# cwchenwang/outdoor-nerf-depth

Hardware: AMD Instinct MI355X
Metric: train rays/sec, KITTI 375x1242, 64+128 samples/ray (higher is better)
Workload: dtype bf16 MFMA operands, f32 accumulate / f32 master weights

## Files before the change

outdoor_nerf_depth_amd/csrc/nerfpp_common.h:

```cpp
#pragma once
#include <stdint.h>
#ifdef NERFPP_PROBES
#include <stdlib.h>
#endif

namespace nerfpp {

constexpr int WIDTH = 256;
constexpr int FRAG_BYTES = 1024;
constexpr int BLK_FRAGS = 16;
constexpr int DIR_REF = 27;
constexpr int DIRW = 32;
constexpr int N_NET = 2;

__host__ __device__ constexpr int pe_dim(int net) { return net == 0 ? 3 : 4; }
__host__ __device__ constexpr int pe_ref_ch(int net) { return net == 0 ? 63 : 84; }
__host__ __device__ constexpr int kpe(int net) { return net == 0 ? 4 : 6; }
__host__ __device__ constexpr int kpew(int net) { return kpe(net) * 16; }

enum RefTensor { RT_L0 = 0, RT_SIGMA = 8, RT_REMAP = 9, RT_RGB0 = 10, RT_RGB1 = 11, RT_COUNT = 12 };
__host__ __device__ constexpr int ref_out(int t) {
  return t < 8 ? 256 : t == RT_SIGMA ? 1 : t == RT_REMAP ? 256 : t == RT_RGB0 ? 128 : 3;
}
__host__ __device__ constexpr int ref_in(int net, int t) {
// ... 19 lines not shown
__host__ __device__ constexpr int fs_nkc(int net, int s) {
  return s == FS_L0 ? kpe(net) : s == FS_L5 ? kpe(net) + 16 : s == FS_REMAP ? 0 : s < FS_REMAP ? 16
       : s == FS_SIG ? 16 : s == FS_RGB0 ? 20 : 16;
}
constexpr int DERIVED_WC = 128 * 256;
constexpr int DERIVED_FLOATS = DERIVED_WC + 128;
__host__ __device__ constexpr int fs_frags(int net, int s) { return fs_nob(s) * fs_nkc(net, s); }
__host__ __device__ constexpr int fs_frag_off(int net, int s) {
  int off = 0;
  for (int i = 0; i < s; ++i) off += fs_frags(net, i);
  return off;
}
__host__ __device__ constexpr int fs_bias_off(int s) {
  int off = 0;
  for (int i = 0; i < s; ++i) off += fs_nob(i) * 32;
  return off;
}
__host__ __device__ constexpr int fwd_frags(int net) { return fs_frag_off(net, FS_COUNT); }
constexpr int FWD_BIAS_FLOATS = fs_bias_off(FS_COUNT);
static_assert(fwd_frags(0) % BLK_FRAGS == 0 && fwd_frags(1) % BLK_FRAGS == 0, "block aligned");

enum BwdStage { BS_DG = 0, BS_DR = 1, BS_DH7 = 2, BS_COUNT = 10 };
__host__ __device__ constexpr int bs_nob(int s) { return s == BS_DG ? 4 : 8; }
__host__ __device__ constexpr int bs_nkc(int s) { return s == BS_DG ? 4 : s == BS_DR ? 0 : s == BS_DH7 ? 10 : 16; }
__host__ __device__ constexpr int bs_frags(int s) { return bs_nob(s) * bs_nkc(s); }
__host__ __device__ constexpr int bs_frag_off(int s) {
  int off = 0;
  for (int i = 0; i < s; ++i) off += bs_frags(i);
  return off;
}
constexpr int BWD_FRAGS = bs_frag_off(BS_COUNT);
static_assert(BWD_FRAGS % BLK_FRAGS == 0, "block aligned");
__host__ __device__ constexpr int bs_layer(int s) { return 10 - s; }

__host__ __device__ constexpr int w_planes(int P) { return P == 1 ? 1 : 2; }
__host__ __device__ constexpr int a_planes(int P) { return P == 2 ? 2 : 1; }
__host__ __device__ constexpr size_t fwd_stream_bytes(int net, int P) { return (size_t)fwd_frags(net) * FRAG_BYTES * w_planes(P); }
__host__ __device__ constexpr size_t bwd_stream_bytes(int P) { return (size_t)BWD_FRAGS * FRAG_BYTES * w_planes(P); }

__host__ __device__ constexpr int kslot(int c, int hi, int t) { return 16 * c + 8 * (t >> 2) + 4 * hi + (t & 3); }
__host__ __device__ constexpr int dfeat(int ob, int hi, int r) { return ob * 32 + (r & 3) + 8 * (r >> 2) + 4 * hi; }

__host__ __device__ constexpr int pe_ref_of_lane_slot(int D, int hi, int m) {
  const int nf = 10 * D;
  if (m < nf) {
    const int k = 5 * hi + m / (2 * D), d = (m % (2 * D)) / 2, s = m & 1;
    return D + k * 2 * D + s * D + d;
  }
  const int id = 2 * hi + (m - nf);
  return (m - nf) < 2 && id < D ? id : -1;
}
__host__ __device__ constexpr int dir_ref_of_lane_slot(int hi, int m) {
  if (m < 12) {
    const int k = 2 * hi + m / 6, d = (m % 6) / 2, s = m & 1;
    return 3 + k * 6 + s * 3 + d;
  }
  const int id = 2 * hi + (m - 12);
  return (m - 12) < 2 && id < 3 ? id : -1;
}
__host__ __device__ constexpr int feat_hi(int f) { return ((f % 16) / 4) % 2; }
__host__ __device__ constexpr int feat_m(int f) { return 8 * (f / 16) + 4 * ((f % 16) / 8) + (f % 4); }
__host__ __device__ constexpr int pe_ref_of_feat(int net, int f) { return pe_ref_of_lane_slot(pe_dim(net), feat_hi(f), feat_m(f)); }
__host__ __device__ constexpr int dir_ref_of_feat(int f) { return dir_ref_of_lane_slot(feat_hi(f), feat_m(f)); }

enum Tensor {
  T_X = 0, T_H0 = 1,  T_R = 9, T_G = 10, T_DIRX = 11,
// ... 211 lines not shown
```

outdoor_nerf_depth_amd/csrc/nerfpp_mlp.hip:

```cpp
#include <hip/hip_runtime.h>
#include <math.h>
#include <stdint.h>
#include <type_traits>
#include <utility>
#include "hip_device.h"
#include "nerfpp_common.h"
#include "nerfpp_kernels.h"

#ifdef NERFPP_PROBES
#include "nerfpp_mlp_probes.h"
#else
namespace nerfpp { namespace probe {
constexpr int STAMP_BYTES = 0;
__device__ __forceinline__ void stamp(int, int, int, int, uint32_t) {}
__device__ __forceinline__ void dump_stamps(uint32_t, int, int) {}
}}
#endif

namespace nerfpp {

using hipdev::bf16x8, hipdev::bf16x2, hipdev::f16x8, hipdev::f16x2, hipdev::f32x2, hipdev::f32x4, hipdev::f32x8, hipdev::f32x16;
using hipdev::u32x4, hipdev::s16x2, hipdev::s16x8, hipdev::glds16xN_saddr;
#define LDS_AS __attribute__((address_space(3)))

template <int P> struct Frag { bf16x8 v[a_planes(P)]; };

extern __shared__ __attribute__((aligned(16))) char smem[];

enum { PIPE_RING = 1, PIPE_ROLES = 2 };

__device__ __forceinline__ uint32_t lds_base_addr() { return (uint32_t)(uintptr_t)(LDS_AS char*)smem; }

template <int P, int NW, int MODE, int NBUF, int BF = BLK_FRAGS>
struct WeightPipe {
  static constexpr int BLKF = BF;
  static constexpr int BLK_BYTES = BF * P * FRAG_BYTES;
  static constexpr int SHARE = MODE == PIPE_ROLES ? BF * P : BF * P / NW;
  static constexpr int AHEAD = NBUF - 1;
  static_assert(AHEAD >= 1 && AHEAD <= 3 && (AHEAD - 1) * SHARE < 63, "ring depth");
  const char* g;
  uint32_t stamp_off = 0;
  int nblk, cur, step, wave, lane;
  int slot_cur, slot_issue, next_issue;
  uint32_t lds_base;
  __device__ __forceinline__ void init(const void* stream, int nblk_, int wave_, int lane_) {
    g = (const char*)stream; nblk = nblk_; cur = 0; step = 0; wave = wave_; lane = lane_;
    slot_cur = 0; slot_issue = 0; next_issue = 0;
    lds_base = lds_base_addr();
#pragma unroll
    for (int b = 0; b < AHEAD; ++b) issue();
  }
  static constexpr bool TRICKLE = MODE == PIPE_RING && AHEAD >= 2;
  int pend_blk = -1, pend_slot = 0;
  __device__ __forceinline__ void issue_frags(int blk, int slot, int f0, int f1) {
    if (MODE == PIPE_ROLES && wave != 0) return;
    const int w0 = MODE == PIPE_ROLES ? 0 : wave * SHARE;
    const char* sb = g + (size_t)blk * BLK_BYTES + (size_t)w0 * FRAG_BYTES;
    const uint32_t dst = lds_base + slot * BLK_BYTES + w0 * FRAG_BYTES;
#pragma unroll
    for (int f = f0; f < f1; f += 4) {
      const int n = f1 - f < 4 ? f1 - f : 4;
      const char* a = sb + f * FRAG_BYTES;
      const uint32_t d = dst + f * FRAG_BYTES;
      if (n == 4) glds16xN_saddr<4>(a, (uint32_t)lane * 16u, d);
      else if (n == 3) glds16xN_saddr<3>(a, (uint32_t)lane * 16u, d);
      else if (n == 2) glds16xN_saddr<2>(a, (uint32_t)lane * 16u, d);
      else glds16xN_saddr<1>(a, (uint32_t)lane * 16u, d);
    }
  }
  __device__ __forceinline__ bool claim(int& blk, int& slot) {
    blk = next_issue; slot = slot_issue;
    ++next_issue;
    slot_issue = slot_issue + 1 == NBUF ? 0 : slot_issue + 1;
    return blk < nblk;
  }
  __device__ __forceinline__ void issue() {
    int blk, slot;
    if (!claim(blk, slot)) return;
    static_assert(SHARE == 2 || SHARE % 4 == 0, "per-wave fragment count");
    issue_frags(blk, slot, 0, SHARE);
  }
  __device__ __forceinline__ void trickle(int i, int n) {
    if constexpr (TRICKLE) {
      if (pend_blk < 0) return;
      issue_frags(pend_blk, pend_slot, SHARE * i / n, SHARE * (i + 1) / n);
    }
  }
  __device__ __forceinline__ void wait_counted() {
    const int younger = nblk - 1 - step < AHEAD - 1 ? nblk - 1 - step : AHEAD - 1;
    if (AHEAD >= 3 && younger >= 2) asm volatile("s_waitcnt vmcnt(%0)" ::"n"(2 * SHARE) : "memory");
    else if (AHEAD >= 2 && younger == 1) asm volatile("s_waitcnt vmcnt(%0)" ::"n"(SHARE) : "memory");
// ... 73 lines not shown
          const f16x8 bf = __builtin_bit_cast(f16x8, b[blk * KPB + kl].v[0]);
#pragma unroll
          for (int g = 0; g < G; ++g) acc[ob + g] = __builtin_amdgcn_mfma_f32_32x32x16_f16(__builtin_bit_cast(f16x8, wh[g]), bf, acc[ob + g], 0, 0, 0);
#pragma unroll
          for (int g = 0; g < G; ++g) acc[ob + g] = __builtin_amdgcn_mfma_f32_32x32x16_f16(__builtin_bit_cast(f16x8, wl[g]), bf, acc[ob + g], 0, 0, 0);
          pipe.trickle(kl * UPB + ob / G, KPB * UPB);
        }
      } else {
#pragma unroll
        for (int ob = 0; ob < NOB; ++ob) {
          mfma_p<P>(acc[ob], l + (kl * NOB + ob) * w_planes(P) * FRAG_BYTES, b[blk * KPB + kl]);
          if (UPB == 2 && (ob & 3) == 3) pipe.trickle(kl * 2 + (ob >> 2), KPB * 2);
        }
        if (UPB == 1) pipe.trickle(kl, KPB);
      }
    }
    hook(blk);
    const int live_kl = LIVE - blk * KPB < KPB ? (LIVE - blk * KPB < 0 ? 0 : LIVE - blk * KPB) : KPB;
    constexpr int W = w_planes(P), D = P == 1 ? LDS_PREFETCH : LDS_PREFETCH_SPLIT;
    const int N = NOB * live_kl;
    if (N < D) continue;
#pragma unroll
    for (int i = 0; i < D; ++i) __builtin_amdgcn_sched_group_barrier(0x100, W, 0);
#pragma unroll
    for (int i = 0; i < N - D; ++i) {
      __builtin_amdgcn_sched_group_barrier(0x008, W, 0);
      __builtin_amdgcn_sched_group_barrier(0x100, W, 0);
    }
#pragma unroll
    for (int i = 0; i < D; ++i) __builtin_amdgcn_sched_group_barrier(0x008, W, 0);
  }
}

template <int P>
__device__ __forceinline__ void set_slot(Frag<P>& f, int t, float v) {
  if constexpr (P == 3) {
    f16x8 q = __builtin_bit_cast(f16x8, f.v[0]);
    q[t] = (_Float16)v;
    f.v[0] = __builtin_bit_cast(bf16x8, q);
    return;
  }
  const __bf16 h = (__bf16)v;
  f.v[0][t] = h;
  if constexpr (P == 2) f.v[1][t] = (__bf16)(v - (float)h);
}
template <int P>
__device__ __forceinline__ uint4 saved_image(const uint4 regs) {
  if constexpr (P == 3) {
    const f32x8 f = __builtin_convertvector(__builtin_bit_cast(f16x8, regs), f32x8);
    return __builtin_bit_cast(uint4, __builtin_convertvector(f, bf16x8));
  } else return regs;
}
template <int P>
__device__ __forceinline__ Frag<P> zero_frag() {
  Frag<P> f;
#pragma unroll
  for (int p = 0; p < a_planes(P); ++p)
#pragma unroll
    for (int t = 0; t < 8; ++t) f.v[p][t] = (__bf16)0.f;
  return f;
}

template <int N, int P>
__device__ __forceinline__ void stash_frags(char* base, int lane, const Frag<P> (&f)[N]) {
#pragma unroll
  for (int c = 0; c < N; ++c)
#pragma unroll
    for (int p = 0; p < a_planes(P); ++p) *(uint4*)(base + ((c * a_planes(P) + p) * 64 + lane) * 16) = *(const uint4*)&f[c].v[p];
}
template <int N, int P>
__device__ __forceinline__ void unstash_frags(const char* base, int lane, Frag<P> (&f)[N]) {
#pragma unroll
  for (int c = 0; c < N; ++c)
#pragma unroll
    for (int p = 0; p < a_planes(P); ++p) *(uint4*)&f[c].v[p] = *(const uint4*)(base + ((c * a_planes(P) + p) * 64 + lane) * 16);
}

template <int P>
__device__ __forceinline__ uint32_t pack2(float a, float b) {
  const f32x2 v = {a, b};
  if constexpr (P == 3) return __builtin_bit_cast(uint32_t, __builtin_convertvector(v, f16x2));
  else return __builtin_bit_cast(uint32_t, __builtin_convertvector(v, bf16x2));
}

template <int NOB, int P>
__device__ __forceinline__ uint4 acc_to_frags_relu_bits(const f32x16 (&acc)[NOB], Frag<P> (&h)[2 * NOB]) {
  static_assert(P == 1 || P == 3, "one operand plane");
  uint32_t m[4] = {0, 0, 0, 0};
#pragma unroll
  for (int ob = 0; ob < NOB; ++ob)
#pragma unroll
    for (int hh = 0; hh < 2; ++hh) {
      u32x4 d;
#pragma unroll
      for (int w = 0; w < 4; ++w) d[w] = pack2<P>(acc[ob][8 * hh + 2 * w], acc[ob][8 * hh + 2 * w + 1]);
#pragma unroll
      for (int w = 0; w < 4; ++w) {
        const int j = (ob & 1) * 8 + hh * 4 + w;
        asm("v_and_or_b32 %0, %1, %2, %0" : "+v"(m[ob >> 1]) : "v"(d[w] >> j), "s"(0x80008000u >> j));
      }
      const s16x8 zero = {0, 0, 0, 0, 0, 0, 0, 0};
      h[2 * ob + hh].v[0] = __builtin_bit_cast(bf16x8, __builtin_elementwise_max(__builtin_bit_cast(s16x8, d), zero));
    }
  return make_uint4(m[0], m[1], m[2], m[3]);
}

template <int N, int P>
__device__ __forceinline__ void zero_invalid(Frag<P> (&f)[N], bool valid) {
#pragma unroll
  for (int c = 0; c < N; ++c)
#pragma unroll
    for (int p = 0; p < a_planes(P); ++p) {
      u32x4 d = __builtin_bit_cast(u32x4, f[c].v[p]);
#pragma unroll
      for (int w = 0; w < 4; ++w) d[w] = valid ? d[w] : 0u;
      f[c].v[p] = __builtin_bit_cast(bf16x8, d);
    }
}

template <int NOB>
__device__ __forceinline__ void init_bias_lds(f32x16 (&acc)[NOB], uint32_t lds_off_bytes, int hi) {
  LDS_AS char* base = (LDS_AS char*)smem;
#pragma unroll
  for (int ob = 0; ob < NOB; ++ob) {
#pragma unroll
    for (int q = 0; q < 4; ++q) {
      const f32x4 v = *(LDS_AS f32x4*)(base + lds_off_bytes + (ob * 32 + hi * 16 + 4 * q) * 4);
      acc[ob][4 * q] = v[0]; acc[ob][4 * q + 1] = v[1]; acc[ob][4 * q + 2] = v[2]; acc[ob][4 * q + 3] = v[3];
    }
  }
}
template <int NOB>
__device__ __forceinline__ void init_zero(f32x16 (&acc)[NOB]) {
#pragma unroll
  for (int ob = 0; ob < NOB; ++ob)
#pragma unroll
    for (int r = 0; r < 16; ++r) acc[ob][r] = 0.f;
}

__device__ __forceinline__ void store_nt16(char* gptr, const uint4 v) {
  const u32x4 vv = {v.x, v.y, v.z, v.w};
  __builtin_nontemporal_store(vv, (u32x4*)gptr);
}

constexpr int REGION_MASK = 16 * FRAG_BYTES;
constexpr int REGION_BYTES = REGION_MASK + 1024;

__device__ __forceinline__ char* frag_addr(__bf16* base, int ld, size_t wave_row0, int c, int lane) {
  const size_t blk = (wave_row0 >> 5) * (size_t)(ld >> 4) + (size_t)c;
  return (char*)base + blk * FRAG_BYTES + ((((lane & 31) << 1) | (lane >> 5)) << 4);
}
template <int P>
__device__ __forceinline__ void store_chunk(__bf16* base, size_t plane, int ld, size_t wave_row0, int lane, int c, const Frag<P>& f, int np = a_planes(P)) {
#pragma unroll
  for (int p = 0; p < a_planes(P); ++p)
    if (p < np) store_nt16(frag_addr(base + p * plane, ld, wave_row0, c, lane), saved_image<P>(*(const uint4*)&f.v[p]));
}
template <int NCH, int P>
__device__ __forceinline__ void save_frags(__bf16* base, size_t plane, int ld, size_t wave_row0, int lane, const Frag<P> (&h)[NCH], int np = a_planes(P)) {
  __builtin_amdgcn_sched_barrier(0);
#pragma unroll
  for (int c = 0; c < NCH; ++c) store_chunk<P>(base, plane, ld, wave_row0, lane, c, h[c], np);
  __builtin_amdgcn_sched_barrier(0);
}

template <int NCH, int P>
__device__ __forceinline__ void handoff_write(char* region, int lane, const Frag<P> (&h)[NCH]) {
  static_assert(a_planes(P) == 1, "one plane");
#pragma unroll
  for (int c = 0; c < NCH; ++c) *(uint4*)(region + (c * 64 + lane) * 16) = *(const uint4*)&h[c].v[0];
}
template <int P>
__device__ __forceinline__ void handoff_flush_one(const char* region, int lane, __bf16* base, int ld, size_t row0, int cr, int ct) {
  static_assert(a_planes(P) == 1, "one plane");
  store_nt16(frag_addr(base, ld, row0, ct, lane), saved_image<P>(*(const uint4*)(region + (cr * 64 + lane) * 16)));
}
template <int P>
__device__ __forceinline__ void handoff_flush_chunks(const char* region, int lane, __bf16* base, int ld, size_t row0, int c0, int n) {
#pragma unroll 4
  for (int c = c0; c < c0 + n; ++c) handoff_flush_one<P>(region, lane, base, ld, row0, c, c);
}

template <int NOB>
__device__ __forceinline__ void mask_to_frags(const f32x16 (&acc)[NOB], const uint4 bits, Frag<1> (&dz)[2 * NOB]) {
  const uint32_t act[4] = {~bits.x, ~bits.y, ~bits.z, ~bits.w};
#pragma unroll
  for (int ob = 0; ob < NOB; ++ob)
#pragma unroll
    for (int hh = 0; hh < 2; ++hh) {
      u32x4 d;
#pragma unroll
      for (int w = 0; w < 4; ++w) d[w] = pack2<1>(acc[ob][8 * hh + 2 * w], acc[ob][8 * hh + 2 * w + 1]);
#pragma unroll
      for (int w = 0; w < 4; ++w) {
        const int j = (ob & 1) * 8 + hh * 4 + w;
        const s16x2 keep = __builtin_bit_cast(s16x2, act[ob >> 1] << j) >> (s16x2){15, 15};
        d[w] &= __builtin_bit_cast(uint32_t, keep);
      }
      dz[2 * ob + hh].v[0] = __builtin_bit_cast(bf16x8, d);
    }
}

template <int NET>
__device__ __forceinline__ void sample_point(const MlpGeom& gm, size_t row, int S, float (&x)[4], float (&vd)[3],
                                             float* depth_real) {
#pragma clang fp contract(off)
  const int ray = (int)(row / S);
  const float ox = gm.ray_o[ray * 3], oy = gm.ray_o[ray * 3 + 1], oz = gm.ray_o[ray * 3 + 2];
  const float dx = gm.ray_d[ray * 3], dy = gm.ray_d[ray * 3 + 1], dz = gm.ray_d[ray * 3 + 2];
  const float z = gm.z[row];
  const float dd = dx * dx + dy * dy + dz * dz;
  const float inv_n = 1.f / sqrtf(dd);
  vd[0] = dx * inv_n; vd[1] = dy * inv_n; vd[2] = dz * inv_n;
  if (NET == 0) {
    x[0] = ox + z * dx; x[1] = oy + z * dy; x[2] = oz + z * dz; x[3] = 0.f;
    *depth_real = 0.f;
  } else {
    const float d1 = -(dx * ox + dy * oy + dz * oz) / dd;
    const float mx = ox + d1 * dx, my = oy + d1 * dy, mz = oz + d1 * dz;
    const float pmn = sqrtf(mx * mx + my * my + mz * mz);
    const float d2 = sqrtf(1.f - pmn * pmn) * inv_n;
    const float sx = ox + (d1 + d2) * dx, sy = oy + (d1 + d2) * dy, sz = oz + (d1 + d2) * dz;
    float ax = oy * sz - oz * sy, ay = oz * sx - ox * sz, az = ox * sy - oy * sx;
    const float an = 1.f / sqrtf(ax * ax + ay * ay + az * az);
    ax *= an; ay *= an; az *= an;
    const float phi = asinf(pmn), theta = asinf(pmn * z);
    float sn, cs;
    sincosf(phi - theta, &sn, &cs);
    const float cx = ay * sz - az * sy, cy = az * sx - ax * sz, cz = ax * sy - ay * sx;
    const float dt = (ax * sx + ay * sy + az * sz) * (1.f - cs);
    float nx = sx * cs + cx * sn + ax * dt, ny = sy * cs + cy * sn + ay * dt, nz = sz * cs + cz * sn + az * dt;
    const float nn = 1.f / sqrtf(nx * nx + ny * ny + nz * nz);
    x[0] = nx * nn; x[1] = ny * nn; x[2] = nz * nn; x[3] = z;
// ... 91 lines not shown
  static constexpr int REGION = W;
  static constexpr int STASH = REGION + (ROLES ? REGION_BYTES : 0);
  static constexpr int BIAS = STASH + NW * kpe(NET) * a_planes(P) * 1024;
  static constexpr int TOTAL = BIAS + FWD_BIAS_FLOATS * 4;
};
template <int NW>
struct BwdLds {
  static constexpr int BF = BLK_FRAGS, NBUF = 4;
  static constexpr int W = NBUF * BF * FRAG_BYTES;
  static constexpr int REGION = W;
  static constexpr int MASKS = REGION + REGION_BYTES;
  static constexpr int TOTAL = MASKS + 2 * NW * 1024;
};

template <int NET, int P, int NW, bool TRAIN>
__device__ __forceinline__ void mlp_fwd_body(const MlpFwdArgs& a, const int bid) {
  using LD = FwdLds<NET, P, NW, TRAIN>;
  static_assert((P == 1 || P == 3) && LD::ROLES == TRAIN, "split-bf16 runs mlp_fwd_body_split");
  constexpr int KPE = kpe(NET);
  const int lane = threadIdx.x & 63, wave = __builtin_amdgcn_readfirstlane(threadIdx.x >> 6);
  const int hi = lane >> 5;
  const size_t row_raw = (size_t)bid * (NW * 32) + wave * 32 + (lane & 31);
  const bool valid = row_raw < (size_t)a.rows;
  const size_t row = valid ? row_raw : (size_t)a.rows - 1;
  const size_t plane_rows = a.rows_padded;
  const size_t wrow0 = (size_t)bid * (NW * 32) + wave * 32;
  const bool loader = TRAIN && wave == 0, partner = TRAIN && wave == 1;
  const bool tail = wrow0 + 32 > (size_t)a.rows;
  char* region = smem + LD::REGION;
  char* pe_stash = smem + LD::STASH + wave * (KPE * 1024);
  const size_t nblk32 = a.rows_padded / 32;
  uint4* mask_out = a.masks + (wrow0 / 32) * 64 + lane;

  WeightPipe<w_planes(P), NW, LD::MODE, LD::NBUF, LD::BF> pipe;
  pipe.stamp_off = LD::TOTAL;
  pipe.init(a.w_stream, fwd_frags(NET) / LD::BF, wave, lane);
  constexpr int H = NW >= 5 ? 4 : NW - 1, Q = (16 + H - 1) / H, CPB = LD::BF / 8;
  constexpr int RMASK = REGION_MASK;
  for (int i = threadIdx.x; i < FWD_BIAS_FLOATS / 4; i += NW * 64)
    *(float4*)(smem + LD::BIAS + i * 16) = ((const float4*)a.bias)[i];
  asm volatile("s_waitcnt vmcnt(0) lgkmcnt(0)" ::: "memory");
  __builtin_amdgcn_s_barrier();
  auto bias_init8 = [&](f32x16 (&acc_)[8], int off) { init_bias_lds<8>(acc_, LD::BIAS + off * 4, hi); };
  auto bias_init4 = [&](f32x16 (&acc_)[4], int off) { init_bias_lds<4>(acc_, LD::BIAS + off * 4, hi); };
  auto bias_init1 = [&](f32x16 (&acc_)[1], int off) { init_bias_lds<1>(acc_, LD::BIAS + off * 4, hi); };
  const size_t tile_row0 = wrow0 - (size_t)wave * 32;
  auto flush = [&](int blk, auto nch_c, __bf16* base, int ld, int mask_stage) __attribute__((always_inline)) {
    if constexpr (TRAIN) {
      constexpr int NCH = decltype(nch_c)::value;
      if (blk == 0 && wave >= 1 && wave <= H) {
#pragma unroll
        for (int c = 0; c < NCH; ++c)
          if ((c % H) == wave - 1) handoff_flush_chunks<P>(region, lane, base, ld, tile_row0, c, 1);
        if (partner && mask_stage >= 0)
          mask_out[(size_t)mask_stage * nblk32 * 64 - 64] = *(const uint4*)(region + RMASK + lane * 16);
      }
    }
  };
  auto finish_h = [&](Frag<P> (&frags)[16], uint4 bits, int mask_stage) __attribute__((always_inline)) {
    if constexpr (!TRAIN) return;
    if (tail) zero_invalid(frags, valid);
    if (loader) *(uint4*)(region + RMASK + lane * 16) = bits;
    else mask_out[(size_t)mask_stage * nblk32 * 64] = bits;
  };
  auto psave_hc = [&](int blk, const Frag<P> (&frags)[16], __bf16* base, int mask_stage, auto cpb_c) __attribute__((always_inline)) {
    constexpr int CPBH = decltype(cpb_c)::value;
    if constexpr (TRAIN) {
// ... 41 lines not shown
  Frag<P> pe[KPE];
  encode_point<NET, P>(x, hi, pe);
  if constexpr (TRAIN) {
    Frag<P> df0[2];
    encode_dir<P>(vd, hi, df0);
    if (tail) { zero_invalid(pe, valid); zero_invalid(df0, valid); }
    if (loader) {
      Frag<P> xd[KPE + 2];
#pragma unroll
      for (int c = 0; c < KPE; ++c) xd[c] = pe[c];
      xd[KPE] = df0[0]; xd[KPE + 1] = df0[1];
      handoff_write<KPE + 2, P>(region, lane, xd);
    } else {
      save_frags<KPE, P>(a.ws.t[T_X], plane_rows * kpew(NET), kpew(NET), wrow0, lane, pe);
      save_frags<2, P>(a.ws.t[T_DIRX], plane_rows * 32, 32, wrow0, lane, df0);
    }
  }
  auto flush_xd = [&](int blk) __attribute__((always_inline)) {
    if constexpr (TRAIN) {
      if (blk == 0 && wave >= 1 && wave <= H) {
#pragma unroll
        for (int c = 0; c < KPE + 2; ++c)
          if ((c % H) == wave - 1) {
            if (c < KPE) handoff_flush_one<P>(region, lane, a.ws.t[T_X], kpew(NET), tile_row0, c, c);
            else handoff_flush_one<P>(region, lane, a.ws.t[T_DIRX], 32, tile_row0, c, c - KPE);
          }
      }
    }
  };
  stash_frags<KPE, P>(pe_stash, lane, pe);

  f32x16 acc[8];
  Frag<P> h[16];
  bias_init8(acc, fs_bias_off(FS_L0));
  stage_gemm<8, KPE, P>(pipe, acc, pe, HOOK(flush_xd(blk)));
  {
    const uint4 bits = acc_to_frags_relu_bits<8, P>(acc, h);
    finish_h(h, bits, 0);
  }
  for (int l = 1; l <= 4; ++l) {
    bias_init8(acc, fs_bias_off(FS_L0) + l * 256);
    stage_gemm<8, 16, P>(pipe, acc, h, HOOK(psave_h(blk, h, a.ws.t[T_H0 + l - 1], l - 1)));
    const uint4 bits = acc_to_frags_relu_bits<8, P>(acc, h);
    finish_h(h, bits, l);
  }
  {
    Frag<P> in5[KPE + 16];
    {
      Frag<P> pe2[KPE];
      unstash_frags<KPE, P>(pe_stash, lane, pe2);
#pragma unroll
      for (int c = 0; c < KPE; ++c) in5[c] = pe2[c];
    }
#pragma unroll
    for (int c = 0; c < 16; ++c) in5[KPE + c] = h[c];
    bias_init8(acc, fs_bias_off(FS_L5));
    stage_gemm<8, KPE + 16, P>(pipe, acc, in5, HOOK(psave_h(blk, h, a.ws.t[T_H0 + 4], 4)));
    const uint4 bits = acc_to_frags_relu_bits<8, P>(acc, h);
    finish_h(h, bits, 5);
  }
  for (int l = 6; l <= 7; ++l) {
    bias_init8(acc, fs_bias_off(FS_L0) + l * 256);
    stage_gemm<8, 16, P>(pipe, acc, h, HOOK(psave_h(blk, h, a.ws.t[T_H0 + l - 1], l - 1)));
    const uint4 bits = acc_to_frags_relu_bits<8, P>(acc, h);
    finish_h(h, bits, l);
  }
  f32x16 acc1[1];
  bias_init1(acc1, fs_bias_off(FS_SIG));
  constexpr int SIG_BLKS = P == 1 ? 1 : 0;
  stage_gemm<1, 16, P>(pipe, acc1, h, HOOK(if constexpr (P == 1) psave_hc(blk, h, a.ws.t[T_H0 + 7], 7, IC(3))));
  const float sigma_raw = acc1[0][0];
  Frag<P> g[8];
  {
    Frag<P> in[20];
#pragma unroll
    for (int c = 0; c < 16; ++c) in[c] = h[c];
    Frag<P> df[2];
    encode_dir<P>(vd, hi, df);
    in[16] = df[0]; in[17] = df[1]; in[18] = zero_frag<P>(); in[19] = zero_frag<P>();
    f32x16 acc4[4];
    bias_init4(acc4, fs_bias_off(FS_RGB0));
    stage_gemm<4, 20, P, 18>(pipe, acc4, in, HOOK(psave_hc(blk + SIG_BLKS, h, a.ws.t[T_H0 + 7], 7, IC(P == 1 ? 3 : 2))));
    const uint4 bits = acc_to_frags_relu_bits<4, P>(acc4, g);
    save(std::integral_constant<int, 8>{}, a.ws.t[T_G], 128, g, true, bits, 8);
  }
  {
    Frag<P> in[16];
#pragma unroll
    for (int c = 0; c < 8; ++c) in[c] = g[c];
#pragma unroll
    for (int c = 8; c < 16; ++c) in[c] = zero_frag<P>();
    bias_init1(acc1, fs_bias_off(FS_RGB1));
    stage_gemm<1, 16, P, 8>(pipe, acc1, in, HOOK(flush(blk, IC(8), a.ws.t[T_G], 128, 8)));
  }
  if (valid && hi == 0) {
    float4 o;
    o.x = 1.f / (1.f + expf(-acc1[0][0]));
    o.y = 1.f / (1.f + expf(-acc1[0][1]));
// ... 21 lines not shown
  const size_t tile_row0 = wrow0 - (size_t)wave * 32;
  const size_t nblk32 = a.rows_padded / 32;
  const uint32_t lds0 = lds_base_addr();

  auto issue_masks = [&](int mstage) __attribute__((always_inline)) {
    if (loader && mstage >= 0) {
      static_assert(NW % 4 == 0, "groups of four");
      const char* sb = (const char*)(a.masks + ((size_t)mstage * nblk32 + (size_t)bid * NW) * 64);
#pragma unroll
      for (int w = 0; w < NW; w += 4) glds16xN_saddr<4>(sb + w * 1024, (uint32_t)lane * 16u, lds0 + LD::MASKS + ((mstage & 1) * NW + w) * 1024);
    }
  };
  auto get_mask = [&](int mstage) __attribute__((always_inline)) -> uint4 {
    return *(const uint4*)(smem + LD::MASKS + ((mstage & 1) * NW + wave) * 1024 + lane * 16);
  };
  auto psave = [&](int blk, auto nch_c, const auto& frags, __bf16* base, int ld) __attribute__((always_inline)) {
    constexpr int NCH = decltype(nch_c)::value, HMAX = NW >= 5 ? 4 : NW - 1, HN = NCH / 4 < HMAX ? NCH / 4 : HMAX;
    constexpr int Q = (NCH + HN - 1) / HN, CPB = LD::BF / 8;
    if (a.skip_dz7 && base == a.ws.t[T_DZ0 + 7]) return;
    if (loader) {
      if (blk == 0) handoff_write<NCH, P>(region, lane, frags);
    } else {
      if (CPB * blk < NCH) {
#pragma unroll
        for (int i = 0; i < CPB; ++i)
          store_chunk<P>(base, plane_rows * ld, ld, wrow0, lane, CPB * blk + i, frags[CPB * blk + i]);
      }
      if (wave <= HN && blk == 2) handoff_flush_chunks<P>(region, lane, base, ld, tile_row0, Q * (wave - 1), Q);
    }
  };

  issue_masks(8);
  issue_masks(7);
  WeightPipe<P, NW, PIPE_ROLES, LD::NBUF, LD::BF> pipe;
  pipe.stamp_off = LD::TOTAL;
  pipe.init(a.w_stream, BWD_FRAGS / LD::BF, wave, lane);

  float4 d = ((const float4*)a.d_out)[row];
  if (!valid) d = make_float4(0.f, 0.f, 0.f, 0.f);
  auto save_dp_ds = [&](const float4& dd, size_t r0) __attribute__((always_inline)) {
    Frag<P> t[2];
    t[0] = zero_frag<P>(); t[1] = zero_frag<P>();
    if (hi == 0) { set_slot<P>(t[0], 0, dd.x); set_slot<P>(t[0], 1, dd.y); set_slot<P>(t[0], 2, dd.z); }
    save_frags<2, P>(a.ws.t[T_DP], plane_rows * 32, 32, r0, lane, t);
    t[0] = zero_frag<P>();
    if (hi == 0) set_slot<P>(t[0], 0, dd.w);
    save_frags<2, P>(a.ws.t[T_DS], plane_rows * DSG_LD, DSG_LD, r0, lane, t);
  };
  {
    const size_t rr = row_raw - 32;
    const bool ok = partner && rr < (size_t)a.rows;
    float4 d0 = make_float4(0.f, 0.f, 0.f, 0.f);
    if (ok) d0 = ((const float4*)a.d_out)[rr];
    if (!loader) save_dp_ds(d, wrow0);
    if (partner) save_dp_ds(d0, wrow0 - 32);
  }

  Frag<P> dg[8];
  {
    Frag<P> in[4];
#pragma unroll
    for (int c = 0; c < 4; ++c) in[c] = zero_frag<P>();
    if (hi == 0) { set_slot<P>(in[0], 0, d.x); set_slot<P>(in[0], 1, d.y); set_slot<P>(in[0], 2, d.z); }
    f32x16 acc4[4];
    init_zero<4>(acc4);
    stage_gemm<4, 4, P, 1>(pipe, acc4, in, NoHook{});
    mask_to_frags<4>(acc4, get_mask(8), dg);
  }
  f32x16 acc[8];
  Frag<P> dz[16];
  {
    Frag<P> in[10];
#pragma unroll
    for (int c = 0; c < 8; ++c) in[c] = dg[c];
    in[8] = zero_frag<P>(); in[9] = zero_frag<P>();
    if (hi == 0) set_slot<P>(in[8], 0, d.w);
    init_zero<8>(acc);
    stage_gemm<8, 10, P, 9>(pipe, acc, in, HOOK(psave(blk, IC(8), dg, a.ws.t[T_DG], DSG_LD); if (blk == 0) issue_masks(6)));
    mask_to_frags<8>(acc, get_mask(7), dz);
  }
  for (int l = 7; l >= 1; --l) {
    init_zero<8>(acc);
    stage_gemm<8, 16, P>(pipe, acc, dz, HOOK(psave(blk, IC(16), dz, a.ws.t[T_DZ0 + l], 256); if (blk == 0) issue_masks(l - 2)));
    mask_to_frags<8>(acc, get_mask(l - 1), dz);
  }
  save_frags<16, P>(a.ws.t[T_DZ0], plane_rows * 256, 256, wrow0, lane, dz);
  probe::dump_stamps(LD::TOTAL, wave, lane);
}

}
#include "nerfpp_mlp_split.h"
namespace nerfpp {

template <int P, int NW, bool TRAIN>
__global__ __launch_bounds__(NW * 64, (NW == 8 ? 2 : 1)) void mlp_fwd_pair_kernel(MlpFwdArgs a0, MlpFwdArgs a1, int tiles0) {
  if constexpr (P == 2) {
    const bool fg = (int)blockIdx.x < tiles0;
    const bool hi_only = TRAIN && !(fg ? a0.save_lo : a1.save_lo);
    if (fg) { if (hi_only) mlp_fwd_body_split<0, NW, TRAIN, TRAIN>(a0, (int)blockIdx.x); else mlp_fwd_body_split<0, NW, TRAIN, false>(a0, (int)blockIdx.x); }
    else { if (hi_only) mlp_fwd_body_split<1, NW, TRAIN, TRAIN>(a1, (int)blockIdx.x - tiles0); else mlp_fwd_body_split<1, NW, TRAIN, false>(a1, (int)blockIdx.x - tiles0); }
  } else {
    if ((int)blockIdx.x < tiles0) mlp_fwd_body<0, P, NW, TRAIN>(a0, (int)blockIdx.x);
    else mlp_fwd_body<1, P, NW, TRAIN>(a1, (int)blockIdx.x - tiles0);
  }
}
template <int P, int NW>
__global__ __launch_bounds__(NW * 64, (P == 1 ? 2 : 1)) void mlp_bwd_pair_kernel(MlpBwdArgs a0, MlpBwdArgs a1, int tiles0) {
  if constexpr (P == 2) {
    if ((int)blockIdx.x < tiles0) mlp_bwd_body_split<0, NW>(a0, (int)blockIdx.x);
    else mlp_bwd_body_split<1, NW>(a1, (int)blockIdx.x - tiles0);
  } else {
    if ((int)blockIdx.x < tiles0) mlp_bwd_body<0, NW>(a0, (int)blockIdx.x);
    else mlp_bwd_body<1, NW>(a1, (int)blockIdx.x - tiles0);
  }
}

}

// ... 70 lines not shown
```

Baseline: 497,500.

## Reorder weight blocks into output-block groups to overlap activation conversion with MFMA

Adds a grouped fragment order for bf16 trunk stages, so each weight block covers one half of the output blocks. The loader gathers blocks through a constant run table. A new stage_gemm_groups finishes the lower four output blocks early and converts them (ReLU/mask packing) while the next stage's MFMAs run, with sched_group_barrier interleaving VALU work into the MFMA stream. This applies to both the forward training trunk and the backward dz chain, hiding the serial accumulator-to-fragment conversion between layers. The cost is double-buffered fragment arrays (more register pressure) and more complex scheduling and save logic.

```diff
diff --git a/outdoor_nerf_depth_amd/csrc/nerfpp_common.h b/outdoor_nerf_depth_amd/csrc/nerfpp_common.h
--- a/outdoor_nerf_depth_amd/csrc/nerfpp_common.h
+++ b/outdoor_nerf_depth_amd/csrc/nerfpp_common.h
@@ -75,6 +75,61 @@
 constexpr int BWD_FRAGS = bs_frag_off(BS_COUNT);
 static_assert(BWD_FRAGS % BLK_FRAGS == 0, "block aligned");
 __host__ __device__ constexpr int bs_layer(int s) { return 10 - s; }
+
+constexpr int GROUP_OBS = 4;
+__host__ __device__ constexpr bool stage_grouped(int nob, int nkc) { return nob == 2 * GROUP_OBS && nkc > 0 && nkc % 4 == 0; }
+__host__ __device__ constexpr int group_frag(int nkc, int b, int p) {
+  const int bpg = nkc / 4;
+  return (4 * (b % bpg) + p / GROUP_OBS) * 8 + GROUP_OBS * (b / bpg) + p % GROUP_OBS;
+}
+__host__ __device__ constexpr int fwd_block_frag(int net, int blk, int p) {
+  for (int s = 0, off = 0; s < FS_COUNT; off += fs_frags(net, s), ++s)
+    if (blk * BLK_FRAGS >= off && blk * BLK_FRAGS < off + fs_frags(net, s) && stage_grouped(fs_nob(s), fs_nkc(net, s)))
+      return off + group_frag(fs_nkc(net, s), blk - off / BLK_FRAGS, p);
+  return blk * BLK_FRAGS + p;
+}
+__host__ __device__ constexpr int bwd_block_frag(int blk, int p) {
+  for (int s = 0, off = 0; s < BS_COUNT; off += bs_frags(s), ++s)
+    if (blk * BLK_FRAGS >= off && blk * BLK_FRAGS < off + bs_frags(s) && stage_grouped(bs_nob(s), bs_nkc(s)))
+      return off + group_frag(bs_nkc(s), blk - off / BLK_FRAGS, p);
+  return blk * BLK_FRAGS + p;
+}
+enum BlockMap { MAP_LINEAR = -1, MAP_FWD_FG = 0, MAP_FWD_BG = 1, MAP_BWD = 2 };
+__host__ __device__ constexpr int map_blocks(int m) { return (m == MAP_BWD ? BWD_FRAGS : fwd_frags(m)) / BLK_FRAGS; }
+__host__ __device__ constexpr int map_frag(int m, int blk, int p) { return m == MAP_BWD ? bwd_block_frag(blk, p) : fwd_block_frag(m, blk, p); }
+constexpr bool map_stage_is_bijection(int m, int off, int n) {
+  if (n == 0) return true;
+  if (off % BLK_FRAGS != 0 || n % BLK_FRAGS != 0) return false;
+  bool seen[512] = {};
+  if (n > 512) return false;
+  for (int blk = off / BLK_FRAGS; blk < (off + n) / BLK_FRAGS; ++blk)
+    for (int p = 0, prev = 0; p < BLK_FRAGS; ++p) {
+      const int f = map_frag(m, blk, p) - off;
+      if (f < 0 || f >= n || seen[f]) return false;
+      if (p % 4 != 0 && f != prev + 1) return false;
+      seen[f] = true;
+      prev = f;
+    }
+  return true;
+}
+constexpr bool map_is_bijection(int m) {
+  const int ns = m == MAP_BWD ? (int)BS_COUNT : (int)FS_COUNT;
+  for (int s = 0; s < ns; ++s)
+    if (!map_stage_is_bijection(m, m == MAP_BWD ? bs_frag_off(s) : fs_frag_off(m, s), m == MAP_BWD ? bs_frags(s) : fs_frags(m, s))) return false;
+  return true;
+}
+static_assert(map_is_bijection(MAP_FWD_FG) && map_is_bijection(MAP_FWD_BG) && map_is_bijection(MAP_BWD),
+              "group order: a block of a stage reads that stage's fragments, each once");
+static_assert(stage_grouped(8, fs_nkc(0, FS_L0)) && stage_grouped(8, fs_nkc(0, FS_L5)) && !stage_grouped(8, fs_nkc(1, FS_L0)) &&
+              !stage_grouped(8, fs_nkc(1, FS_L5)) && !stage_grouped(8, bs_nkc(BS_DH7)) && stage_grouped(8, bs_nkc(3)) &&
+              !stage_grouped(fs_nob(FS_RGB0), fs_nkc(0, FS_RGB0)), "grouped stages");
+template <int M> struct RunTable { uint32_t off[map_blocks(M)][4]; };
+template <int M> constexpr RunTable<M> make_run_table() {
+  RunTable<M> t{};
+  for (int blk = 0; blk < map_blocks(M); ++blk)
+    for (int r = 0; r < 4; ++r) t.off[blk][r] = (uint32_t)map_frag(M, blk, 4 * r) * FRAG_BYTES;
+  return t;
+}
 
 __host__ __device__ constexpr int w_planes(int P) { return P == 1 ? 1 : 2; }
 __host__ __device__ constexpr int a_planes(int P) { return P == 2 ? 2 : 1; }
diff --git a/outdoor_nerf_depth_amd/csrc/nerfpp_mlp.hip b/outdoor_nerf_depth_amd/csrc/nerfpp_mlp.hip
--- a/outdoor_nerf_depth_amd/csrc/nerfpp_mlp.hip
+++ b/outdoor_nerf_depth_amd/csrc/nerfpp_mlp.hip
@@ -31,9 +31,19 @@
 
 __device__ __forceinline__ uint32_t lds_base_addr() { return (uint32_t)(uintptr_t)(LDS_AS char*)smem; }
 
-template <int P, int NW, int MODE, int NBUF, int BF = BLK_FRAGS>
+[[maybe_unused]] static __constant__ const RunTable<MAP_FWD_FG> RUNS_FWD_FG = make_run_table<MAP_FWD_FG>();
+[[maybe_unused]] static __constant__ const RunTable<MAP_FWD_BG> RUNS_FWD_BG = make_run_table<MAP_FWD_BG>();
+[[maybe_unused]] static __constant__ const RunTable<MAP_BWD> RUNS_BWD = make_run_table<MAP_BWD>();
+template <int M>
+__device__ __forceinline__ const uint32_t* run_offsets(int blk) {
+  if constexpr (M == MAP_FWD_FG) return RUNS_FWD_FG.off[blk];
+  else if constexpr (M == MAP_FWD_BG) return RUNS_FWD_BG.off[blk];
+  else return RUNS_BWD.off[blk];
+}
+
+template <int P, int NW, int MODE, int NBUF, int BF = BLK_FRAGS, int MAP = MAP_LINEAR>
 struct WeightPipe {
-  static constexpr int BLKF = BF;
+  static constexpr int BLKF = BF, MAP_ID = MAP;
   static constexpr int BLK_BYTES = BF * P * FRAG_BYTES;
   static constexpr int SHARE = MODE == PIPE_ROLES ? BF * P : BF * P / NW;
   static constexpr int AHEAD = NBUF - 1;
@@ -57,6 +67,13 @@
     const int w0 = MODE == PIPE_ROLES ? 0 : wave * SHARE;
     const char* sb = g + (size_t)blk * BLK_BYTES + (size_t)w0 * FRAG_BYTES;
     const uint32_t dst = lds_base + slot * BLK_BYTES + w0 * FRAG_BYTES;
+    if constexpr (MAP != MAP_LINEAR) {
+      static_assert(MODE == PIPE_ROLES && P == 1 && BF == BLK_FRAGS, "group order: the loader of the bf16 roles pipe");
+      const uint32_t* run = run_offsets<MAP>(blk);
+#pragma unroll
+      for (int r = 0; r < 4; ++r) glds16xN_saddr<4>(g + run[r], (uint32_t)lane * 16u, dst + r * 4 * FRAG_BYTES);
+      return;
+    }
 #pragma unroll
     for (int f = f0; f < f1; f += 4) {
       const int n = f1 - f < 4 ? f1 - f : 4;
@@ -196,6 +213,40 @@
   }
 }
 
+template <int P, bool PEND, int DS0, int DS1, int IV, int NKC, typename Pipe, typename Init, typename Work, typename Hook>
+__device__ __forceinline__ void stage_gemm_groups(Pipe& pipe, f32x16 (&acc)[8], const Frag<P> (&b)[NKC], const Init& init, const Work& work,
+                                                  const Hook& hook) {
+  static_assert(P == 1 && Pipe::BLKF == BLK_FRAGS && Pipe::MAP_ID != MAP_LINEAR && stage_grouped(8, NKC), "a bf16 stage in group order");
+  constexpr int BPG = NKC / 4, INIT1 = PEND ? 2 : BPG - 1;
+  static_assert(!PEND || BPG >= 4, "the upper out-blocks of the previous stage are converted in blocks 0 and 1, one of this stage's per block of group 1");
+#pragma unroll
+  for (int blk = 0; blk < 2 * BPG; ++blk) {
+    const char* l = pipe.acquire();
+    if (blk == 0) init(0);
+    if (blk == INIT1) init(1);
+    work(blk);
+#pragma unroll
+    for (int p = 0; p < BLK_FRAGS; ++p) {
+      const int f = group_frag(NKC, blk, p);
+      mfma_p<P>(acc[f % 8], l + p * FRAG_BYTES, b[f / 8]);
+    }
+    hook(blk);
+    const int conv_obs = (PEND && blk < 2 ? 2 : 0) + (blk >= BPG ? (BPG >= 4 ? (blk - BPG < 4 ? 1 : 0) : 4 / BPG) : 0);
+    const int NV = 2 * conv_obs + IV * ((blk == 0) + (blk == INIT1));
+    const int nds = DS0 * (blk == 0) + DS1 * (blk == INIT1);
+    constexpr int D = LDS_PREFETCH, N = BLK_FRAGS;
+#pragma unroll
+    for (int i = 0; i < nds + D; ++i) __builtin_amdgcn_sched_group_barrier(0x100, 1, 0);
+#pragma unroll
+    for (int i = 0; i < N; ++i) {
+      __builtin_amdgcn_sched_group_barrier(0x008, 1, 0);
+#pragma unroll
+      for (int v = 0; v < NV; ++v) __builtin_amdgcn_sched_group_barrier(0x002, 1, 0);
+      if (i < N - D) __builtin_amdgcn_sched_group_barrier(0x100, 1, 0);
+    }
+  }
+}
+
 template <int P>
 __device__ __forceinline__ void set_slot(Frag<P>& f, int t, float v) {
   if constexpr (P == 3) {
@@ -247,30 +298,46 @@
   else return __builtin_bit_cast(uint32_t, __builtin_convertvector(v, bf16x2));
 }
 
+template <int P>
+__device__ __forceinline__ void ob_to_frags_relu_bits(const f32x16& acc, const int ob, Frag<P>* h, uint32_t& m) {
+  static_assert(P == 1 || P == 3, "one operand plane");
+#pragma unroll
+  for (int hh = 0; hh < 2; ++hh) {
+    u32x4 d;
+#pragma unroll
+    for (int w = 0; w < 4; ++w) d[w] = pack2<P>(acc[8 * hh + 2 * w], acc[8 * hh + 2 * w + 1]);
+#pragma unroll
+    for (int w = 0; w < 4; ++w) {
+      const int j = (ob & 1) * 8 + hh * 4 + w;
+      asm("v_and_or_b32 %0, %1, %2, %0" : "+v"(m) : "v"(d[w] >> j), "s"(0x80008000u >> j));
+    }
+    const s16x8 zero = {0, 0, 0, 0, 0, 0, 0, 0};
+    h[hh].v[0] = __builtin_bit_cast(bf16x8, __builtin_elementwise_max(__builtin_bit_cast(s16x8, d), zero));
+  }
+}
 template <int NOB, int P>
 __device__ __forceinline__ uint4 acc_to_frags_relu_bits(const f32x16 (&acc)[NOB], Frag<P> (&h)[2 * NOB]) {
-  static_assert(P == 1 || P == 3, "one operand plane");
   uint32_t m[4] = {0, 0, 0, 0};
 #pragma unroll
-  for (int ob = 0; ob < NOB; ++ob)
-#pragma unroll
-    for (int hh = 0; hh < 2; ++hh) {
-      u32x4 d;
-#pragma unroll
-      for (int w = 0; w < 4; ++w) d[w] = pack2<P>(acc[ob][8 * hh + 2 * w], acc[ob][8 * hh + 2 * w + 1]);
-#pragma unroll
-      for (int w = 0; w < 4; ++w) {
-        const int j = (ob & 1) * 8 + hh * 4 + w;
-        asm("v_and_or_b32 %0, %1, %2, %0" : "+v"(m[ob >> 1]) : "v"(d[w] >> j), "s"(0x80008000u >> j));
-      }
-      const s16x8 zero = {0, 0, 0, 0, 0, 0, 0, 0};
-      h[2 * ob + hh].v[0] = __builtin_bit_cast(bf16x8, __builtin_elementwise_max(__builtin_bit_cast(s16x8, d), zero));
-    }
+  for (int ob = 0; ob < NOB; ++ob) ob_to_frags_relu_bits<P>(acc[ob], ob, &h[2 * ob], m[ob >> 1]);
   return make_uint4(m[0], m[1], m[2], m[3]);
 }
 
 template <int N, int P>
 __device__ __forceinline__ void zero_invalid(Frag<P> (&f)[N], bool valid) {
+#pragma unroll
+  for (int c = 0; c < N; ++c)
+#pragma unroll
+    for (int p = 0; p < a_planes(P); ++p) {
+      u32x4 d = __builtin_bit_cast(u32x4, f[c].v[p]);
+#pragma unroll
+      for (int w = 0; w < 4; ++w) d[w] = valid ? d[w] : 0u;
+      f[c].v[p] = __builtin_bit_cast(bf16x8, d);
+    }
+}
+
+template <int N, int P>
+__device__ __forceinline__ void zero_invalid_n(Frag<P>* f, bool valid) {
 #pragma unroll
   for (int c = 0; c < N; ++c)
 #pragma unroll
@@ -294,6 +361,24 @@
     }
   }
 }
+__device__ __forceinline__ void init_bias_lds_group(f32x16 (&acc)[8], int g, uint32_t lds_off_bytes, int hi) {
+  LDS_AS char* base = (LDS_AS char*)smem;
+#pragma unroll
+  for (int o = 0; o < GROUP_OBS; ++o) {
+    const int ob = GROUP_OBS * g + o;
+#pragma unroll
+    for (int q = 0; q < 4; ++q) {
+      const f32x4 v = *(LDS_AS f32x4*)(base + lds_off_bytes + (ob * 32 + hi * 16 + 4 * q) * 4);
+      acc[ob][4 * q] = v[0]; acc[ob][4 * q + 1] = v[1]; acc[ob][4 * q + 2] = v[2]; acc[ob][4 * q + 3] = v[3];
+    }
+  }
+}
+__device__ __forceinline__ void init_zero_group(f32x16 (&acc)[8], int g) {
+#pragma unroll
+  for (int o = 0; o < GROUP_OBS; ++o)
+#pragma unroll
+    for (int r = 0; r < 16; ++r) acc[GROUP_OBS * g + o][r] = 0.f;
+}
 template <int NOB>
 __device__ __forceinline__ void init_zero(f32x16 (&acc)[NOB]) {
 #pragma unroll
@@ -333,6 +418,12 @@
   static_assert(a_planes(P) == 1, "one plane");
 #pragma unroll
   for (int c = 0; c < NCH; ++c) *(uint4*)(region + (c * 64 + lane) * 16) = *(const uint4*)&h[c].v[0];
+}
+template <int NCH, int P>
+__device__ __forceinline__ void handoff_write_part(char* region, int lane, const Frag<P>* h, int c0) {
+  static_assert(a_planes(P) == 1, "one plane");
+#pragma unroll
+  for (int c = c0; c < c0 + NCH; ++c) *(uint4*)(region + (c * 64 + lane) * 16) = *(const uint4*)&h[c].v[0];
 }
 template <int P>
 __device__ __forceinline__ void handoff_flush_one(const char* region, int lane, __bf16* base, int ld, size_t row0, int cr, int ct) {
@@ -345,24 +436,26 @@
   for (int c = c0; c < c0 + n; ++c) handoff_flush_one<P>(region, lane, base, ld, row0, c, c);
 }
 
+__device__ __forceinline__ void ob_mask_to_frags(const f32x16& acc, const int ob, const uint32_t act, Frag<1>* dz) {
+#pragma unroll
+  for (int hh = 0; hh < 2; ++hh) {
+    u32x4 d;
+#pragma unroll
+    for (int w = 0; w < 4; ++w) d[w] = pack2<1>(acc[8 * hh + 2 * w], acc[8 * hh + 2 * w + 1]);
+#pragma unroll
+    for (int w = 0; w < 4; ++w) {
+      const int j = (ob & 1) * 8 + hh * 4 + w;
+      const s16x2 keep = __builtin_bit_cast(s16x2, act << j) >> (s16x2){15, 15};
+      d[w] &= __builtin_bit_cast(uint32_t, keep);
+    }
+    dz[hh].v[0] = __builtin_bit_cast(bf16x8, d);
+  }
+}
 template <int NOB>
 __device__ __forceinline__ void mask_to_frags(const f32x16 (&acc)[NOB], const uint4 bits, Frag<1> (&dz)[2 * NOB]) {
   const uint32_t act[4] = {~bits.x, ~bits.y, ~bits.z, ~bits.w};
 #pragma unroll
-  for (int ob = 0; ob < NOB; ++ob)
-#pragma unroll
-    for (int hh = 0; hh < 2; ++hh) {
-      u32x4 d;
-#pragma unroll
-      for (int w = 0; w < 4; ++w) d[w] = pack2<1>(acc[ob][8 * hh + 2 * w], acc[ob][8 * hh + 2 * w + 1]);
-#pragma unroll
-      for (int w = 0; w < 4; ++w) {
-        const int j = (ob & 1) * 8 + hh * 4 + w;
-        const s16x2 keep = __builtin_bit_cast(s16x2, act[ob >> 1] << j) >> (s16x2){15, 15};
-        d[w] &= __builtin_bit_cast(uint32_t, keep);
-      }
-      dz[2 * ob + hh].v[0] = __builtin_bit_cast(bf16x8, d);
-    }
+  for (int ob = 0; ob < NOB; ++ob) ob_mask_to_frags(acc[ob], ob, act[ob >> 1], &dz[2 * ob]);
 }
 
 template <int NET>
@@ -520,7 +613,8 @@
   const size_t nblk32 = a.rows_padded / 32;
   uint4* mask_out = a.masks + (wrow0 / 32) * 64 + lane;
 
-  WeightPipe<w_planes(P), NW, LD::MODE, LD::NBUF, LD::BF> pipe;
+  constexpr bool GROUPS = TRAIN && P == 1;
+  WeightPipe<w_planes(P), NW, LD::MODE, LD::NBUF, LD::BF, GROUPS ? (NET == 0 ? MAP_FWD_FG : MAP_FWD_BG) : MAP_LINEAR> pipe;
   pipe.stamp_off = LD::TOTAL;
   pipe.init(a.w_stream, fwd_frags(NET) / LD::BF, wave, lane);
   constexpr int H = NW >= 5 ? 4 : NW - 1, Q = (16 + H - 1) / H, CPB = LD::BF / 8;
@@ -628,6 +722,97 @@
 
   f32x16 acc[8];
   Frag<P> h[16];
+  if constexpr (GROUPS) {
+    Frag<P> h2[16];
+    uint32_t m[4] = {0, 0, 0, 0};
+    auto conv = [&](Frag<P>* t, int ob0, int n) __attribute__((always_inline)) {
+#pragma unroll
+      for (int ob = ob0; ob < ob0 + n; ++ob) {
+        if ((ob & 1) == 0) m[ob >> 1] = 0;
+        ob_to_frags_relu_bits<P>(acc[ob], ob, t + 2 * ob, m[ob >> 1]);
+      }
+    };
+    auto bits_out = [&](int mask_stage) __attribute__((always_inline)) {
+      const uint4 bits = make_uint4(m[0], m[1], m[2], m[3]);
+      if (loader) *(uint4*)(region + RMASK + lane * 16) = bits;
+      else mask_out[(size_t)mask_stage * nblk32 * 64] = bits;
+    };
+    auto upper_now = [&](Frag<P>* t, int mask_stage) __attribute__((always_inline)) {
+      conv(t, 4, 4);
+      if (tail) zero_invalid_n<8>(t + 8, valid);
+      bits_out(mask_stage);
+    };
+    auto psave_late = [&](int blk, const Frag<P>* t, __bf16* base, int mask_stage) __attribute__((always_inline)) {
+      const bool skip = mask_stage == 0 && a.skip_h0;
+      if (skip) {
+        if (partner && blk == 2) mask_out[(size_t)mask_stage * nblk32 * 64 - 64] = *(const uint4*)(region + RMASK + lane * 16);
+      } else if (loader) {
+        if (blk < 2) handoff_write_part<8, P>(region, lane, t, 8 * blk);
+      } else {
+        if (blk < 8) {
+          store_chunk<P>(base, plane_rows * 256, 256, wrow0, lane, 2 * blk, t[2 * blk]);
+          store_chunk<P>(base, plane_rows * 256, 256, wrow0, lane, 2 * blk + 1, t[2 * blk + 1]);
+        }
+        if (wave <= H && blk == 2) handoff_flush_chunks<P>(region, lane, base, 256, tile_row0, Q * (wave - 1), Q);
+        if (partner && blk == 2) mask_out[(size_t)mask_stage * nblk32 * 64 - 64] = *(const uint4*)(region + RMASK + lane * 16);
+      }
+    };
+    auto trunk = [&](const auto& bin, Frag<P>* tin, Frag<P>* tout, int bias_off, int lin) __attribute__((always_inline)) {
+      constexpr int BPG = (int)(sizeof(bin) / sizeof(bin[0])) / 4;
+      stage_gemm_groups<P, true, 16, 16, 0>(pipe, acc, bin,
+        [&](int g) __attribute__((always_inline)) { init_bias_lds_group(acc, g, LD::BIAS + bias_off * 4, hi); },
+        [&](int blk) __attribute__((always_inline)) {
+          if (blk < 2) conv(tin, 4 + 2 * blk, 2);
+          if (blk >= BPG && blk < BPG + 4) conv(tout, blk - BPG, 1);
+        },
+        [&](int blk) __attribute__((always_inline)) {
+          if (blk < 2 && tail) zero_invalid_n<4>(tin + 8 + 4 * blk, valid);
+          if (blk == 1) bits_out(lin);
+          if (blk >= BPG && blk < BPG + 4 && tail) zero_invalid_n<2>(tout + 2 * (blk - BPG), valid);
+          psave_late(blk, tin, a.ws.t[T_H0 + lin], lin);
+        });
+    };
+    if constexpr (stage_grouped(8, KPE)) {
+      stage_gemm_groups<P, false, 16, 16, 0>(pipe, acc, pe,
+        [&](int g) __attribute__((always_inline)) { init_bias_lds_group(acc, g, LD::BIAS + fs_bias_off(FS_L0) * 4, hi); },
+        [&](int blk) __attribute__((always_inline)) { if (blk == 1) conv(h2, 0, 4); },
+        [&](int blk) __attribute__((always_inline)) { if (blk == 1 && tail) zero_invalid_n<8>(h2, valid); flush_xd(blk); });
+    } else {
+      bias_init8(acc, fs_bias_off(FS_L0));
+      stage_gemm<8, KPE, P>(pipe, acc, pe, HOOK(flush_xd(blk)));
+      conv(h2, 0, 4);
+      if (tail) zero_invalid_n<8>(h2, valid);
+    }
+    for (int l = 1; l <= 3; l += 2) {
+      trunk(h2, h2, h, fs_bias_off(FS_L0) + l * 256, l - 1);
+      trunk(h, h, h2, fs_bias_off(FS_L0) + (l + 1) * 256, l);
+    }
+    {
+      Frag<P> in5[KPE + 16];
+      {
+        Frag<P> pe2[KPE];
+        unstash_frags<KPE, P>(pe_stash, lane, pe2);
+#pragma unroll
+        for (int c = 0; c < KPE; ++c) in5[c] = pe2[c];
+      }
+      if constexpr (stage_grouped(8, KPE + 16)) {
+#pragma unroll
+        for (int c = 0; c < 8; ++c) in5[KPE + c] = h2[c];
+        trunk(in5, in5 + KPE, h, fs_bias_off(FS_L5), 4);
+      } else {
+        upper_now(h2, 4);
+#pragma unroll
+        for (int c = 0; c < 16; ++c) in5[KPE + c] = h2[c];
+        bias_init8(acc, fs_bias_off(FS_L5));
+        stage_gemm<8, KPE + 16, P>(pipe, acc, in5, HOOK(psave_h(blk, h2, a.ws.t[T_H0 + 4], 4)));
+        conv(h, 0, 4);
+        if (tail) zero_invalid_n<8>(h, valid);
+      }
+    }
+    trunk(h, h, h2, fs_bias_off(FS_L0) + 6 * 256, 5);
+    trunk(h2, h2, h, fs_bias_off(FS_L0) + 7 * 256, 6);
+    upper_now(h, 7);
+  } else {
   bias_init8(acc, fs_bias_off(FS_L0));
   stage_gemm<8, KPE, P>(pipe, acc, pe, HOOK(flush_xd(blk)));
   {
@@ -660,6 +845,7 @@
     stage_gemm<8, 16, P>(pipe, acc, h, HOOK(psave_h(blk, h, a.ws.t[T_H0 + l - 1], l - 1)));
     const uint4 bits = acc_to_frags_relu_bits<8, P>(acc, h);
     finish_h(h, bits, l);
+  }
   }
   f32x16 acc1[1];
   bias_init1(acc1, fs_bias_off(FS_SIG));
@@ -747,7 +933,7 @@
 
   issue_masks(8);
   issue_masks(7);
-  WeightPipe<P, NW, PIPE_ROLES, LD::NBUF, LD::BF> pipe;
+  WeightPipe<P, NW, PIPE_ROLES, LD::NBUF, LD::BF, MAP_BWD> pipe;
   pipe.stamp_off = LD::TOTAL;
   pipe.init(a.w_stream, BWD_FRAGS / LD::BF, wave, lane);
 
@@ -792,13 +978,48 @@
     if (hi == 0) set_slot<P>(in[8], 0, d.w);
     init_zero<8>(acc);
     stage_gemm<8, 10, P, 9>(pipe, acc, in, HOOK(psave(blk, IC(8), dg, a.ws.t[T_DG], DSG_LD); if (blk == 0) issue_masks(6)));
-    mask_to_frags<8>(acc, get_mask(7), dz);
-  }
-  for (int l = 7; l >= 1; --l) {
-    init_zero<8>(acc);
-    stage_gemm<8, 16, P>(pipe, acc, dz, HOOK(psave(blk, IC(16), dz, a.ws.t[T_DZ0 + l], 256); if (blk == 0) issue_masks(l - 2)));
-    mask_to_frags<8>(acc, get_mask(l - 1), dz);
-  }
+  }
+  Frag<P> dz2[16];
+  uint32_t pact[4], cact[4];
+  auto read_act = [&](uint32_t (&act)[4], int mstage) __attribute__((always_inline)) {
+    const uint4 bits = get_mask(mstage);
+    act[0] = ~bits.x; act[1] = ~bits.y; act[2] = ~bits.z; act[3] = ~bits.w;
+  };
+  auto conv = [&](Frag<P>* t, const uint32_t (&act)[4], int ob0, int n) __attribute__((always_inline)) {
+#pragma unroll
+    for (int ob = ob0; ob < ob0 + n; ++ob) ob_mask_to_frags(acc[ob], ob, act[ob >> 1], t + 2 * ob);
+  };
+  auto psave_late = [&](int blk, const Frag<P>* t, __bf16* base) __attribute__((always_inline)) {
+    constexpr int HN = NW >= 5 ? 4 : NW - 1, Q = 16 / HN;
+    static_assert(Q * HN == 16, "the helpers share the loader's tile");
+    if (a.skip_dz7 && base == a.ws.t[T_DZ0 + 7]) return;
+    if (loader) {
+      if (blk < 2) handoff_write_part<8, P>(region, lane, t, 8 * blk);
+    } else {
+      store_chunk<P>(base, plane_rows * 256, 256, wrow0, lane, 2 * blk, t[2 * blk]);
+      store_chunk<P>(base, plane_rows * 256, 256, wrow0, lane, 2 * blk + 1, t[2 * blk + 1]);
+      if (wave <= HN && blk == 2) handoff_flush_chunks<P>(region, lane, base, 256, tile_row0, Q * (wave - 1), Q);
+    }
+  };
+  auto dx_stage = [&](const Frag<P> (&bin)[16], Frag<P>* tin, Frag<P>* tout, int l) __attribute__((always_inline)) {
+    stage_gemm_groups<P, true, 0, 1, 4>(pipe, acc, bin,
+      [&](int g) __attribute__((always_inline)) { init_zero_group(acc, g); if (g == 1) read_act(cact, l - 1); },
+      [&](int blk) __attribute__((always_inline)) {
+        if (blk < 2) conv(tin, pact, 4 + 2 * blk, 2);
+        if (blk >= 4) conv(tout, cact, blk - 4, 1);
+      },
+      [&](int blk) __attribute__((always_inline)) { psave_late(blk, tin, a.ws.t[T_DZ0 + l]); if (blk == 0) issue_masks(l - 2); });
+#pragma unroll
+    for (int i = 0; i < 4; ++i) pact[i] = cact[i];
+  };
+  read_act(pact, 7);
+  conv(dz2, pact, 0, 4);
+  for (int l = 7; l >= 3; l -= 2) {
+    dx_stage(dz2, dz2, dz, l);
+    dx_stage(dz, dz, dz2, l - 1);
+  }
+  dx_stage(dz2, dz2, dz, 1);
+  conv(dz, pact, 4, 4);
   save_frags<16, P>(a.ws.t[T_DZ0], plane_rows * 256, 256, wrow0, lane, dz);
   probe::dump_stamps(LD::TOTAL, wave, lane);
 }
```

New measurement: 499,700, median of 6. Within noise of the previous version (+0.5%).
